# hpc4cmb/toast

Hardware: NVIDIA B200
Metric: detector-samples/s per destriper PCG iteration (higher is better)
Workload: dtype f64

## Files before the change

### include/toast_b200.h

```cpp
#ifndef TOAST_B200_H
#define TOAST_B200_H

#include <stddef.h>
#include <stdint.h>

#ifdef __cplusplus
extern "C" {
#endif

typedef struct {
    double start;
    double stop;
    int64_t first;
    int64_t last;
} tb_interval;

enum { TB_MEM_HOST = 0, TB_MEM_DEVICE = 1, TB_MEM_TABLE = 2 };

enum {
    TB_OK = 0,
    TB_ERR_CUDA = 1,
    TB_ERR_NO_DEVICE = 2,
    TB_ERR_ARG = 3,
    TB_ERR_NOT_PRESENT = 4,
// ... 186 lines not shown
    int64_t step_length;
    int64_t nside, n_pix_submap, n_submap;
    int nest, IAU;
    const int64_t *global2local;
    const double *boresight;
    const uint8_t *shared_flags;
    uint8_t shared_flag_mask;
    const uint8_t *solver_flags;
    uint8_t solver_flag_mask;
    const int64_t *pixels;
    const double *weights;
    const double *hwp;
} tb_obs_desc;

tb_obs *tb_obs_create(const tb_obs_desc *desc);
void tb_obs_destroy(tb_obs *obs);

int tb_lhs_pass1(const tb_obs *obs, const double *amplitudes, const uint8_t *amp_flags,
                 double *zmap, int regen, void *stream);
int tb_lhs_pass2(const tb_obs *obs, const double *amplitudes, const uint8_t *amp_flags,
                 const double *binned, double *amplitudes_out, int regen, void *stream);
int tb_obs_sorted_passes(const tb_obs *obs);
int tb_obs_set_pixel_chunks(tb_obs *obs, int64_t n_chunks, const int64_t *pixel_bounds);
int tb_lhs_pass1_chunk(const tb_obs *obs, const double *amplitudes, const uint8_t *amp_flags,
                       double *zmap, int64_t chunk, void *stream);
int tb_lhs_pass2_chunk(const tb_obs *obs, const double *binned, double *amplitudes_out,
                       int64_t chunk, void *stream);
int tb_lhs_pass2_cov(const tb_obs *obs, const double *zmap, const double *cov,
                     double *amplitudes_out, void *stream);
int tb_bx_block_pixels(void);
int tb_obs_blocked(const tb_obs *obs);
int tb_obs_blocked_stats(const tb_obs *obs, int64_t *n_records, int64_t *n_units,
                         int64_t *n_multi_units, int64_t *n_blocks);
int tb_bx_pass1(const tb_obs *obs, const double *amplitudes, const uint8_t *amp_flags,
                double *zmap, int accumulate, int64_t chunk, void *stream);
int tb_bx_pass2(const tb_obs *obs, const double *binned, double *amplitudes_out, int64_t chunk,
                void *stream);
int tb_bx_fused(const tb_obs *obs, const double *amplitudes, const uint8_t *amp_flags,
                const double *cov, double *zmap_scratch, double *amplitudes_out, void *stream);
int tb_rhs_project(const tb_obs *obs, const double *signal, const uint8_t *amp_flags,
                   const double *binned, double *amplitudes_out, int regen, void *stream);
int tb_bin_signal(const tb_obs *obs, const double *signal, double *zmap, int regen,
                  void *stream);

#define TB_PRECOND_TOEPLITZ 1
#define TB_PRECOND_BANDED 2
typedef struct {
    int64_t n_amp;
    int64_t n_seg;
    const int64_t *seg_start;
    const int64_t *seg_len;
    const int64_t *filt_start;
    const int64_t *filt_len;
    const double *filters;
    int64_t n_filter_values;
    int precond_mode;
    const int64_t *prec_start;
    const int64_t *prec_width;
    const double *precond;
    int64_t n_precond_values;
} tb_offset_prior_desc;
typedef struct tb_offset_prior tb_offset_prior;
tb_offset_prior *tb_offset_prior_create(const tb_offset_prior_desc *desc);
void tb_offset_prior_destroy(tb_offset_prior *prior);
int tb_offset_prior_add(const tb_offset_prior *prior, const double *amplitudes_in,
                        const uint8_t *amplitude_flags, double *amplitudes_out, int mem,
// ... 43 lines not shown
```

### toast_b200/csrc/tb_blocked.cu

```cuda
#include <algorithm>

#include "tb_obs.cuh"

using namespace tbd;

namespace tbr {
void sort_pairs_i32(const int32_t *keys_in, int32_t *keys_out, const int32_t *vals_in,
                    int32_t *vals_out, int64_t n, int end_bit, cudaStream_t st);
}

int g_use_bx = 1;

namespace {

#ifndef TB_BX_SHIFT
#define TB_BX_SHIFT 7
#endif
#ifndef TB_BX_CTAS
#define TB_BX_CTAS 4
#endif

constexpr int kBxShift = TB_BX_SHIFT;
constexpr int kBxPix = 1 << kBxShift;
constexpr int kBxUnitMax = 16384;
constexpr int kBxRowBits = 32 - (kBxShift + 12);
static_assert(kBxRowBits >= 1, "pixel | n0 | n1 must fit one int");

template <bool TWO_SLOT>
__global__ void __launch_bounds__(kThreads)
k_bx_keys(const int4 *__restrict__ xrec, int64_t n_rec, int32_t n_blocks, int32_t *__restrict__ keys,
          int32_t *__restrict__ vals, unsigned int *__restrict__ counters ) {
    for (int64_t i = (int64_t)blockIdx.x * kThreads + threadIdx.x; i < n_rec;
         i += (int64_t)gridDim.x * kThreads) {
        const int4 r = xrec[i];
        int32_t key = n_blocks, val = (int32_t)i, key2 = n_blocks, val2 = (int32_t)i | (2 << 30);
        if (r.x == -2 || r.y == -2) atomicAdd(counters + 2, 1u);
        if (r.x >= 0) {
            key = r.x >> kBxShift;
            if (r.y >= 0 && r.y != r.x) {
                val |= (1 << 30);
                key2 = r.y >> kBxShift;
                atomicAdd(counters, 1u);
            }
        } else if (r.y >= 0) {
// ... 61 lines not shown
        const double a0 = g0 ? __ldg(amps + o0 + i) * w0 : 0.0;
        if (paired) {
            const bool g1 = has1 && __ldg(aflags + o1 + i) == 0;
            const double a1 = g1 ? __ldg(amps + o1 + i) * w1 : 0.0;
            double2 *dst = reinterpret_cast<double2 *>(ascaled) + 2 * ((int64_t)row * nad + i);
            dst[0] = make_double2(a0, a1);
            dst[1] = make_double2(g0 ? w0 : 0.0, g1 ? w1 : 0.0);
        } else {
            reinterpret_cast<double2 *>(ascaled)[(int64_t)row * nad + i] =
                make_double2(a0, g0 ? w0 : 0.0);
        }
    }
}

struct BxArgs {
    const int4 *units;
    const int2 *brec;
    const double2 *bqu;
    const double *ascaled;
    double *out;
    const int64_t *amp_offsets;
    int32_t nad, n_det;
    double4 cst;
    const double4 *table;
    double inv_nad;
    int64_t n_pix;
    double *zmap;
    const double *cov;
    int accumulate;
};

constexpr int kBxWarps = kThreads / 32;

struct BxRec {
    int2 r;
    double2 qu;
};
template <bool KEEP_IN_L2>
__device__ __forceinline__ BxRec bx_load(const BxArgs &a, int i, int end, int lane) {
    BxRec x;
    x.r = make_int2(0, -1 - lane);
    x.qu = make_double2(0.0, 0.0);
    if (i < end) {
        x.r = KEEP_IN_L2 ? __ldg(a.brec + i) : __ldcs(a.brec + i);
        x.qu = KEEP_IN_L2 ? __ldg(a.bqu + i) : __ldcs(a.bqu + i);
    }
    return x;
}

struct BxAmp {
    double2 t;
    double2 w;
};
template <bool PAIRED, bool NEED_W>
__device__ __forceinline__ BxAmp bx_gather(const BxArgs &a, int32_t slot) {
    BxAmp g;
    g.t = g.w = make_double2(0.0, 0.0);
    if (slot >= 0) {
        if (PAIRED) {
            const double2 *p = reinterpret_cast<const double2 *>(a.ascaled) + 2 * (int64_t)slot;
            g.t = __ldg(p);
            if (NEED_W) g.w = __ldg(p + 1);
        } else {
            const double2 v = __ldg(reinterpret_cast<const double2 *>(a.ascaled) + slot);
            g.t.x = v.x;
            g.w.x = v.y;
        }
    }
    return g;
}

template <bool UNIFORM>
__device__ __forceinline__ double4 bx_consts(const BxArgs &a, int32_t slot) {
    if (UNIFORM) return a.cst;
    const int row = (int)fast_div((int64_t)(slot < 0 ? 0 : slot), a.inv_nad);
    const double2 *tp = reinterpret_cast<const double2 *>(a.table + row);
    const double2 ca = __ldg(tp), cb = __ldg(tp + 1);
    return make_double4(ca.x, ca.y, cb.x, cb.y);
}

template <bool UNIFORM, bool PAIRED>
__device__ __forceinline__ void bx_acc_step(const BxArgs &a, double *tile, const BxRec &x,
                                            const BxAmp &g, int lane) {
    const int p = x.r.x & (kBxPix - 1);
    const int n0 = (x.r.x >> kBxShift) & 63, n1 = (x.r.x >> (kBxShift + 6)) & 63;
    const double4 c = bx_consts<UNIFORM>(a, x.r.y);
    const double t0 = n0 ? g.t.x : 0.0;
    const double t1 = (PAIRED && n1) ? g.t.y : 0.0;
    const bool contrib = t0 != 0.0 || t1 != 0.0;
    const double v0 = t0 * (c.x * (double)n0) + t1 * (c.y * (double)n1);
    const double v1 = t0 * x.qu.x + t1 * (c.z * x.qu.x - c.w * x.qu.y);
    const double v2 = t0 * x.qu.y + t1 * (c.w * x.qu.x + c.z * x.qu.y);
    const unsigned same = __match_any_sync(0xffffffffu, contrib ? p : kBxPix + lane);
    const int rank = __popc(same & ((1u << lane) - 1u));
    const int rounds = __reduce_max_sync(0xffffffffu, rank);
    double *z = tile + 3 * p;
    if (rounds == 0) {
        if (contrib) {
            z[0] += v0;
            z[1] += v1;
            z[2] += v2;
        }
        __syncwarp();
    } else {
        for (int r = 0; r <= rounds; ++r) {
            if (contrib && rank == r) {
                z[0] += v0;
                z[1] += v1;
                z[2] += v2;
            }
            __syncwarp();
        }
    }
}

template <bool UNIFORM, bool PAIRED, bool KEEP_IN_L2>
__device__ __forceinline__ void bx_accumulate(const BxArgs &a, double *tile, int first, int end,
                                              int lane) {
    if (first >= end) return;
    BxRec A = bx_load<KEEP_IN_L2>(a, first + lane, end, lane);
    BxRec B = bx_load<KEEP_IN_L2>(a, first + 32 + lane, end, lane);
    BxRec C;
    BxAmp gA = bx_gather<PAIRED, false>(a, A.r.y), gB, gC;
    for (int base = first; base < end; base += 96) {
        C = bx_load<KEEP_IN_L2>(a, base + 64 + lane, end, lane);
        gB = bx_gather<PAIRED, false>(a, B.r.y);
        bx_acc_step<UNIFORM, PAIRED>(a, tile, A, gA, lane);
        if (base + 32 >= end) break;
        A = bx_load<KEEP_IN_L2>(a, base + 96 + lane, end, lane);
        gC = bx_gather<PAIRED, false>(a, C.r.y);
        bx_acc_step<UNIFORM, PAIRED>(a, tile, B, gB, lane);
        if (base + 64 >= end) break;
        B = bx_load<KEEP_IN_L2>(a, base + 128 + lane, end, lane);
        gA = bx_gather<PAIRED, false>(a, A.r.y);
        bx_acc_step<UNIFORM, PAIRED>(a, tile, C, gC, lane);
    }
}

template <bool UNIFORM, bool PAIRED>
__device__ __forceinline__ void bx_proj_step(const BxArgs &a, const double *tile, const BxRec &x,
                                             const BxAmp &g, int lane) {
    const int p = x.r.x & (kBxPix - 1);
    const int n0 = (x.r.x >> kBxShift) & 63, n1 = (x.r.x >> (kBxShift + 6)) & 63;
    const double4 c = bx_consts<UNIFORM>(a, x.r.y);
    const double m0 = tile[3 * p], m1 = tile[3 * p + 1], m2 = tile[3 * p + 2];
    double val0 = 0.0, val1 = 0.0;
    if (n0) {
        double sc = (c.x * (double)n0) * m0;
        sc += x.qu.x * m1;
        sc += x.qu.y * m2;
        val0 = (double)n0 * g.t.x - sc * g.w.x;
    }
    if (PAIRED && n1) {
        const double q1 = c.z * x.qu.x - c.w * x.qu.y, u1 = c.w * x.qu.x + c.z * x.qu.y;
        double sc = (c.y * (double)n1) * m0;
        sc += q1 * m1;
        sc += u1 * m2;
        val1 = (double)n1 * g.t.y - sc * g.w.y;
    }
    const Runs rr = find_runs32<8>(x.r.y, lane);
    val0 = seg_sum<8>(val0, rr);
    if (PAIRED) val1 = seg_sum<8>(val1, rr);
    if (rr.is_tail && x.r.y >= 0) {
        const int row = (int)((unsigned)x.r.x >> (kBxShift + 12));
        const int arel = x.r.y - row * a.nad;
        const int d0 = PAIRED ? 2 * row : row;
        if (val0 != 0.0) atomicAdd(a.out + __ldg(a.amp_offsets + d0) + arel, val0);
        if (PAIRED && val1 != 0.0) atomicAdd(a.out + __ldg(a.amp_offsets + d0 + 1) + arel, val1);
    }
}

template <bool UNIFORM, bool PAIRED>
__device__ __forceinline__ void bx_project(const BxArgs &a, const double *tile, int first, int end,
                                           int lane) {
    if (first >= end) return;
    BxRec A = bx_load<false>(a, first + lane, end, lane);
    BxRec B = bx_load<false>(a, first + 32 + lane, end, lane);
    BxRec C;
    BxAmp gA = bx_gather<PAIRED, true>(a, A.r.y), gB, gC;
    for (int base = first; base < end; base += 96) {
        C = bx_load<false>(a, base + 64 + lane, end, lane);
        gB = bx_gather<PAIRED, true>(a, B.r.y);
        bx_proj_step<UNIFORM, PAIRED>(a, tile, A, gA, lane);
        if (base + 32 >= end) break;
        A = bx_load<false>(a, base + 96 + lane, end, lane);
        gC = bx_gather<PAIRED, true>(a, C.r.y);
        bx_proj_step<UNIFORM, PAIRED>(a, tile, B, gB, lane);
        if (base + 64 >= end) break;
        B = bx_load<false>(a, base + 128 + lane, end, lane);
        gA = bx_gather<PAIRED, true>(a, A.r.y);
        bx_proj_step<UNIFORM, PAIRED>(a, tile, C, gC, lane);
    }
}

template <int MODE, bool UNIFORM, bool PAIRED>
__global__ void __launch_bounds__(kThreads, TB_BX_CTAS)
k_bx(const BxArgs a, int64_t n_units) {
    __shared__ __align__(16) double tiles[kBxWarps][3 * kBxPix];
    const int warp = threadIdx.x >> 5, lane = threadIdx.x & 31;
    double *tile = tiles[warp];
    double2 *tile2 = reinterpret_cast<double2 *>(tile);
    const int64_t g_end = 3 * a.n_pix;
    {
        const int64_t ticket = (int64_t)blockIdx.x * kBxWarps + warp;
        if (ticket >= n_units) return;
        const int4 u = __ldg(a.units + ticket);
        const int64_t g0 = (int64_t)u.x * (3 * kBxPix);
        if constexpr (MODE == 1) {
            if (u.z <= u.y) return;
            const double2 *src = reinterpret_cast<const double2 *>(a.zmap + g0);
#pragma unroll 4
            for (int k = lane; k < 3 * kBxPix / 2; k += 32) {
                const int64_t g = g0 + 2 * k;
                double2 v = make_double2(0.0, 0.0);
                if (g + 1 < g_end) v = __ldcs(src + k);
                else if (g < g_end) v.x = __ldcs(a.zmap + g);
                tile2[k] = v;
            }
            __syncwarp();
            bx_project<UNIFORM, PAIRED>(a, tile, u.y, u.z, lane);
        } else {
#pragma unroll 4
            for (int k = lane; k < 3 * kBxPix / 2; k += 32) tile2[k] = make_double2(0.0, 0.0);
            __syncwarp();
            bx_accumulate<UNIFORM, PAIRED, MODE == 2>(a, tile, u.y, u.z, lane);
            __syncwarp();
            if constexpr (MODE == 0) {
                if (u.w == 0 && !a.accumulate) {
                    double2 *dst = reinterpret_cast<double2 *>(a.zmap + g0);
#pragma unroll 4
                    for (int k = lane; k < 3 * kBxPix / 2; k += 32) {
                        const int64_t gg = g0 + 2 * k;
                        if (gg + 1 < g_end) __stcs(dst + k, tile2[k]);
                        else if (gg < g_end) a.zmap[gg] = tile2[k].x;
                    }
                } else {
                    for (int k = lane; k < 3 * kBxPix; k += 32) {
                        const double v = tile[k];
                        if (v != 0.0 && g0 + k < g_end) atomicAdd(a.zmap + g0 + k, v);
                    }
                }
            } else if (u.z > u.y) {
                for (int p = lane; p < kBxPix; p += 32) {
                    const int64_t gp = (int64_t)u.x * kBxPix + p;
                    const double z0 = tile[3 * p], z1 = tile[3 * p + 1], z2 = tile[3 * p + 2];
                    if (gp >= a.n_pix || (z0 == 0.0 && z1 == 0.0 && z2 == 0.0)) continue;
                    const double2 *cm = reinterpret_cast<const double2 *>(a.cov + 6 * gp);
                    const double2 ca = __ldcs(cm), cb = __ldcs(cm + 1), cc = __ldcs(cm + 2);
                    double m0 = 0.0, m1 = 0.0, m2 = 0.0;
                    m0 += ca.x * z0;
                    m0 += ca.y * z1;
                    m1 += ca.y * z0;
                    m0 += cb.x * z2;
                    m2 += cb.x * z0;
                    m1 += cb.y * z1;
                    m1 += cc.x * z2;
                    m2 += cc.x * z1;
                    m2 += cc.y * z2;
                    tile[3 * p] = m0;
                    tile[3 * p + 1] = m1;
                    tile[3 * p + 2] = m2;
                }
                __syncwarp();
                bx_project<UNIFORM, PAIRED>(a, tile, u.y, u.z, lane);
            }
        }
    }
}

__global__ void __launch_bounds__(kThreads)
k_bx_zero_blocks(const int32_t *__restrict__ blocks, int64_t n_pix, double *__restrict__ zmap) {
    const int64_t g0 = (int64_t)__ldg(blocks + blockIdx.x) * (3 * kBxPix);
    for (int k = threadIdx.x; k < 3 * kBxPix; k += kThreads)
        if (g0 + k < 3 * n_pix) zmap[g0 + k] = 0.0;
}

__global__ void __launch_bounds__(kThreads)
k_bx_cov_blocks(const int32_t *__restrict__ blocks, int64_t n_pix, const double *__restrict__ cov,
                double *__restrict__ zmap) {
    const int64_t p0 = (int64_t)__ldg(blocks + blockIdx.x) * kBxPix;
    for (int p = threadIdx.x; p < kBxPix; p += kThreads) {
        const int64_t gp = p0 + p;
        if (gp >= n_pix) continue;
        double *z = zmap + 3 * gp;
        const double z0 = z[0], z1 = z[1], z2 = z[2];
        const double *m = cov + 6 * gp;
        double t0 = 0.0, t1 = 0.0, t2 = 0.0;
        t0 += m[0] * z0;
        t0 += m[1] * z1;
        t1 += m[1] * z0;
        t0 += m[2] * z2;
        t2 += m[2] * z0;
        t1 += m[3] * z1;
        t1 += m[4] * z2;
        t2 += m[4] * z1;
        t2 += m[5] * z2;
        z[0] = t0;
        z[1] = t1;
        z[2] = t2;
    }
}

BxArgs make_args(const tb_obs *obs, const int4 *units) {
    BxArgs a;
    a.units = units;
    a.brec = obs->brec;
    a.bqu = obs->bqu;
    a.ascaled = obs->ascaled;
    a.out = nullptr;
    a.amp_offsets = obs->amp_offsets;
    a.nad = (int32_t)obs->n_amp_det;
    a.n_det = (int)obs->d.n_det;
    a.cst = make_double4(obs->s_const[0], obs->s_const[1], obs->s_const[2], obs->s_const[3]);
    a.table = obs->stable;
    a.inv_nad = 1.0 / (double)obs->n_amp_det;
    a.n_pix = obs->n_local_pix;
    a.zmap = nullptr;
    a.cov = nullptr;
    a.accumulate = 0;
    return a;
}

void row_grid(const tb_obs *obs, dim3 &grid) {
    int64_t gy = (obs->n_amp_det + kThreads * 4 - 1) / (kThreads * 4);
    if (gy < 1) gy = 1;
    if (gy > 65535) gy = 65535;
    grid = dim3((unsigned)obs->n_xrows, (unsigned)gy);
}

void launch_bx_prescale(const tb_obs *obs, const double *amps, const uint8_t *aflags, void *stream) {
    dim3 grid;
    row_grid(obs, grid);
    k_bx_prescale<<<grid, kThreads, 0, (cudaStream_t)stream>>>(
        obs->x_paired, (int)obs->d.n_det, obs->n_amp_det, obs->amp_offsets, obs->det_scale, amps,
        aflags, obs->ascaled);
    TB_CUDA(cudaGetLastError());
    tbr::count_launch();
}

template <int MODE>
void launch_bx(const tb_obs *obs, const BxArgs &a, int64_t n_units, void *stream) {
    if (n_units <= 0) return;
    const int64_t nb = (n_units + kBxWarps - 1) / kBxWarps;
    TB_REQUIRE(nb < 2147483647LL, "grid too large");
    const unsigned g = (unsigned)nb;
    cudaStream_t st = (cudaStream_t)stream;
    static bool configured = false;
    if (!configured) {
        auto prep = [&](const void *f) {
            TB_CUDA(cudaFuncSetAttribute(f, cudaFuncAttributePreferredSharedMemoryCarveout,
                                         (int)cudaSharedmemCarveoutMaxShared));
        };
        prep((const void *)k_bx<MODE, true, true>);
        prep((const void *)k_bx<MODE, true, false>);
        prep((const void *)k_bx<MODE, false, true>);
        prep((const void *)k_bx<MODE, false, false>);
        configured = true;
    }
    if (obs->s_uniform) {
        if (obs->x_paired) k_bx<MODE, true, true><<<g, kThreads, 0, st>>>(a, n_units);
        else k_bx<MODE, true, false><<<g, kThreads, 0, st>>>(a, n_units);
    } else {
        if (obs->x_paired) k_bx<MODE, false, true><<<g, kThreads, 0, st>>>(a, n_units);
        else k_bx<MODE, false, false><<<g, kThreads, 0, st>>>(a, n_units);
    }
    TB_CUDA(cudaGetLastError());
    tbr::count_launch();
}

inline bool bx_ok(const tb_obs *obs) { return g_use_bx && obs != nullptr && obs->brec != nullptr; }

void chunk_units(const tb_obs *obs, int64_t chunk, int64_t &first, int64_t &end) {
    first = 0;
    end = obs->n_bunits;
    if (chunk < 0) return;
    TB_REQUIRE(chunk + 1 < (int64_t)obs->bchunk_unit.size(),
               "bad chunk index (or pixel chunk bounds not aligned to the block size)");
    first = obs->bchunk_unit[chunk];
    end = obs->bchunk_unit[chunk + 1];
}

}

void tb_free_blocked(tb_obs *obs) {
    if (obs->brec) cudaFree(obs->brec);
    if (obs->bqu) cudaFree(obs->bqu);
    if (obs->bunits) cudaFree(obs->bunits);
    if (obs->bunits_single) cudaFree(obs->bunits_single);
    if (obs->bunits_multi) cudaFree(obs->bunits_multi);
    if (obs->bmulti_blocks) cudaFree(obs->bmulti_blocks);
    if (obs->ascaled) cudaFree(obs->ascaled);
    obs->ascaled = nullptr;
    obs->brec = nullptr;
    obs->bqu = nullptr;
    obs->bunits = obs->bunits_single = obs->bunits_multi = nullptr;
    obs->bmulti_blocks = nullptr;
    obs->n_brec = obs->n_bunits = obs->n_bunits_single = obs->n_bunits_multi = 0;
// ... 122 lines not shown
    for (int64_t c = 0; c <= n_chunks; ++c) {
        const int64_t b = pixel_bounds[c];
        if (!(b % kBxPix == 0 || b >= obs->n_local_pix)) {
            obs->bchunk_unit.clear();
            return;
        }
        const int64_t blk = (b + kBxPix - 1) >> kBxShift;
        auto it = std::lower_bound(obs->bunits_host.begin(), obs->bunits_host.end(), blk,
                                   [](const int4 &u, int64_t v) { return (int64_t)u.x < v; });
        cu[c] = (int64_t)(it - obs->bunits_host.begin());
    }
    cu[0] = 0;
    cu[n_chunks] = obs->n_bunits;
    obs->bchunk_unit = cu;
}

extern "C" {

int tb_bx_block_pixels(void) { return kBxPix; }

int tb_obs_blocked(const tb_obs *obs) { return bx_ok(obs) ? 1 : 0; }

int tb_obs_blocked_stats(const tb_obs *obs, int64_t *n_records, int64_t *n_units,
                         int64_t *n_multi_units, int64_t *n_blocks) {
    TB_API_BEGIN
    TB_REQUIRE(obs != nullptr, "NULL observation");
    if (n_records) *n_records = obs->n_brec;
    if (n_units) *n_units = obs->n_bunits;
    if (n_multi_units) *n_multi_units = obs->n_bunits_multi;
    if (n_blocks) *n_blocks = obs->brec ? (obs->n_local_pix + kBxPix - 1) >> kBxShift : 0;
    TB_API_END
}

int tb_bx_pass1(const tb_obs *obs, const double *amplitudes, const uint8_t *amp_flags,
                double *zmap, int accumulate, int64_t chunk, void *stream) {
    TB_API_BEGIN
    tbr::require_device();
    TB_REQUIRE(obs && amplitudes && amp_flags && zmap, "NULL argument");
    TB_REQUIRE(bx_ok(obs), "the observation has no block-ordered crossing list");
    TB_REQUIRE((reinterpret_cast<uintptr_t>(zmap) & 15u) == 0, "zmap must be 16-byte aligned");
    int64_t first, end;
    chunk_units(obs, chunk, first, end);
    if (chunk <= 0) launch_bx_prescale(obs, amplitudes, amp_flags, stream);
    if (!accumulate && obs->n_bmulti_blocks > 0 && chunk <= 0) {
        k_bx_zero_blocks<<<(unsigned)obs->n_bmulti_blocks, kThreads, 0, (cudaStream_t)stream>>>(
            obs->bmulti_blocks, obs->n_local_pix, zmap);
        TB_CUDA(cudaGetLastError());
        tbr::count_launch();
    }
    BxArgs a = make_args(obs, obs->bunits + first);
    a.zmap = zmap;
    a.accumulate = accumulate;
    launch_bx<0>(obs, a, end - first, stream);
    TB_API_END
}

int tb_bx_pass2(const tb_obs *obs, const double *binned, double *amplitudes_out, int64_t chunk,
                void *stream) {
    TB_API_BEGIN
    tbr::require_device();
    TB_REQUIRE(obs && binned && amplitudes_out, "NULL argument");
    TB_REQUIRE(bx_ok(obs), "the observation has no block-ordered crossing list");
    TB_REQUIRE((reinterpret_cast<uintptr_t>(binned) & 15u) == 0, "map must be 16-byte aligned");
    int64_t first, end;
    chunk_units(obs, chunk, first, end);
    BxArgs a = make_args(obs, obs->bunits + first);
// ... 45 lines not shown
```

### toast_b200/csrc/tb_obs.cuh

```cuda
#pragma once

#include <vector>

#include "tb_device.cuh"
#include "tb_runtime.cuh"

using tbd::Views;

struct tb_obs {
    void *blob = nullptr;
    Views V;
    const int64_t *amp_view_off = nullptr;
    const int64_t *amp_offsets = nullptr;
    const int64_t *g2l = nullptr;
    const double *fp = nullptr;
    const double *cal = nullptr;
    const double *eta = nullptr;
    const double *gamma = nullptr;
    const double *det_scale = nullptr;
    tb_obs_desc d;
    int64_t n_amp_det = 0;
    int64_t *tiles = nullptr;
    int64_t n_tiles = 0;
    int32_t *lpix = nullptr;
// ... 8 lines not shown
    int4 *srec = nullptr;
    double2 *squ = nullptr;
    double4 *stable = nullptr;
    double *dscaled = nullptr;
    int64_t n_srec = 0;
    int s_pass2_ok = 0;
    std::vector<int64_t> chunk_rec;
    double *ascaled = nullptr;
    int2 *brec = nullptr;
    double2 *bqu = nullptr;
    int4 *bunits = nullptr;
    int4 *bunits_single = nullptr, *bunits_multi = nullptr;
    int32_t *bmulti_blocks = nullptr;
    int64_t n_brec = 0, n_bunits = 0, n_bunits_single = 0, n_bunits_multi = 0, n_bmulti_blocks = 0;
    int64_t n_local_pix = 0;
    std::vector<int4> bunits_host;
    std::vector<int64_t> bchunk_unit;
    int s_uniform = 0;
    double s_const[4] = {0, 0, 0, 0};
};


constexpr unsigned long long kAmpFlagBits = 0x7FF8000000B200B2ULL;
__device__ __forceinline__ bool amp_is_flagged(double v) {
    return (unsigned long long)__double_as_longlong(v) == kAmpFlagBits;
}

void tb_launch_prescale(const tb_obs *obs, const double *amps, const uint8_t *aflags, void *stream);
void tb_build_row_table(tb_obs *obs);
void tb_build_blocked(tb_obs *obs, cudaStream_t st);
void tb_free_blocked(tb_obs *obs);
void tb_blocked_set_chunks(tb_obs *obs, int64_t n_chunks, const int64_t *pixel_bounds);
extern int g_use_bx;
```

### toast_b200/csrc/tb_solver.cu

```cuda
#include "tb_device.cuh"
#include "tb_runtime.cuh"

using namespace tbd;

#include "tb_obs.cuh"
#include "tb_tma.cuh"

namespace {

struct ObsDev {
    Views V;
    int64_t n_det, n_samp;
    const int64_t *amp_view_off, *amp_offsets, *g2l;
    const double *fp, *cal, *eta, *gamma, *det_scale;
    double inv_step, inv_nps;
    int64_t n_pix_submap;
    tbm::PixCtx ctx;
    double U_sign;
    const double *boresight;
    const uint8_t *shared_flags;
    uint8_t shared_mask;
    const uint8_t *solver_flags;
    uint8_t solver_mask;
    const int64_t *pixels;
// ... 1954 lines not shown
        }
        build_crossings(obs, (cudaStream_t)stream);
    }
    TB_API_END
}

int tb_obs_crossing_stats(const tb_obs *obs, int64_t *n_records, int64_t *n_rows, int *paired) {
    TB_API_BEGIN
    TB_REQUIRE(obs != nullptr, "NULL observation");
    if (n_records) *n_records = obs->xrec ? obs->n_xrec : 0;
    if (n_rows) *n_rows = obs->xrec ? obs->n_xrows : 0;
    if (paired) *paired = obs->xrec ? obs->x_paired : 0;
    TB_API_END
}

int tb_obs_has_compact_pointing(const tb_obs *obs) { return (obs && obs->lpix) ? 1 : 0; }
int tb_obs_has_pair_weights(const tb_obs *obs) { return (obs && obs->lpp) ? 1 : 0; }

extern int tb_peer_ctas_per_sm;
extern int tb_prior_chunk;

int tb_get_option(const char *name) {
    if (name == nullptr) return -1;
    std::string n(name);
    if (n == "tma") return g_use_tma;
    if (n == "compact") return g_use_compact;
    if (n == "pair") return g_use_pair;
    if (n == "pairw") return g_use_pairw;
    if (n == "crossings") return g_use_x;
    if (n == "sorted") return g_use_xs;
    if (n == "sorted2") return g_use_xs2;
    if (n == "peer_ctas") return tb_peer_ctas_per_sm;
    if (n == "blocked") return g_use_bx;
    if (n == "prior_chunk") return tb_prior_chunk;
    return -1;
}

int tb_set_option(const char *name, int value) {
    TB_API_BEGIN
    TB_REQUIRE(name != nullptr, "NULL option name");
    if (std::string(name) == "tma") {
        g_use_tma = value;
    } else if (std::string(name) == "compact") {
        g_use_compact = value;
    } else if (std::string(name) == "pair") {
        g_use_pair = value;
    } else if (std::string(name) == "pairw") {
        g_use_pairw = value;
    } else if (std::string(name) == "crossings") {
        g_use_x = value;
    } else if (std::string(name) == "sorted") {
        g_use_xs = value;
    } else if (std::string(name) == "sorted2") {
        g_use_xs2 = value;
    } else if (std::string(name) == "blocked") {
        g_use_bx = value;
    } else if (std::string(name) == "prior_chunk") {
        TB_REQUIRE(value >= 0, "prior_chunk must be >= 0");
        tb_prior_chunk = value;
    } else if (std::string(name) == "peer_ctas") {
        TB_REQUIRE(value >= 1 && value <= 16, "peer_ctas must be in [1, 16]");
        tb_peer_ctas_per_sm = value;
    } else {
        throw tbr::Error{TB_ERR_ARG, std::string("unknown option: ") + name};
    }
    TB_API_END
}

int tb_lhs_pass1(const tb_obs *obs, const double *amplitudes, const uint8_t *amp_flags,
                 double *zmap, int regen, void *stream) {
    TB_API_BEGIN
    tbr::require_device();
    TB_REQUIRE(obs && amplitudes && amp_flags && zmap, "NULL argument");
    launch_bin<false>(obs, amplitudes, amp_flags, nullptr, zmap, regen, stream);
    TB_API_END
}

int tb_lhs_pass2(const tb_obs *obs, const double *amplitudes, const uint8_t *amp_flags,
                 const double *binned, double *amplitudes_out, int regen, void *stream) {
    TB_API_BEGIN
    tbr::require_device();
    TB_REQUIRE(obs && amp_flags && binned && amplitudes_out, "NULL argument");
    launch_project<false>(obs, amplitudes, amp_flags, nullptr, binned, amplitudes_out, regen,
                          stream);
    TB_API_END
}

int tb_obs_sorted_passes(const tb_obs *obs) {
    if (obs == nullptr) return 0;
// ... 128 lines not shown
```

### toast_b200/lib.py

```python

import ctypes as ct
import os

import numpy as np

HERE = os.path.dirname(os.path.abspath(__file__))
LIB_PATH = os.environ.get("TB_LIB_PATH", os.path.join(HERE, "libtoastb200.so"))

TB_MEM_HOST, TB_MEM_DEVICE, TB_MEM_TABLE = 0, 1, 2
TB_ERR_NO_DEVICE = 2

interval_dtype = np.dtype(
    {
        "names": ["start", "stop", "first", "last"],
        "formats": ["d", "d", "q", "q"],
        "offsets": [0, 8, 16, 24],
    }
)

P = ct.c_void_p
I64 = ct.c_int64
I32 = ct.c_int32
U8 = ct.c_uint8
F64 = ct.c_double
# ... 65 lines not shown
    "tb_stokes_weights_I": (INT, [P, P, I64, P, I64, P, I64, I64, INT, P]),
    "tb_pointing_fused": (INT, [P, P, P, U8, P, P, I64, P, P, I64, P, P, I64, P, P, I64, P, I64,
                                I64, I64, INT, P, P, P, INT, I64, I64, INT, P]),
    "tb_noise_weight": (INT, [P, I64, P, P, I64, P, I64, I64, INT, P]),
    "tb_build_noise_weighted": (INT, [P, I64, P, I64, I64, I64, P, P, I64, P, P, I64, P, P, I64,
                                      P, P, I64, P, U8, P, I64, P, U8, I64, I64, INT, P]),
    "tb_scan_map": (INT, [P, I64, I64, P, INT, I64, I64, P, I64, P, P, I64, P, P, I64, P, P,
                          I64, F64, INT, INT, INT, I64, I64, INT, P]),
    "tb_template_offset_add_to_signal": (INT, [I64, I64, P, P, P, I64, I32, P, I64, P, I64, I64,
                                               INT, P]),
    "tb_template_offset_project_signal": (INT, [I32, P, I64, I32, P, I64, U8, I64, I64, P, P, P,
                                                I64, P, I64, I64, INT, P]),
    "tb_template_offset_apply_diag_precond": (INT, [P, P, P, P, I64, INT, P]),
    "tb_template_offset_add_to_signal_batch": (INT, [I64, P, P, P, P, I64, P, P, I64, P, I64,
                                                     I64, I64, INT, P]),
    "tb_template_offset_project_signal_batch": (INT, [P, P, I64, P, P, I64, U8, I64, P, P, P, P,
                                                      I64, P, I64, I64, I64, INT, P]),
    "tb_cov_apply_diag": (INT, [I64, I64, I64, P, P, INT, P]),
    "tb_cov_accum": (INT, [P, I64, I64, I64, I64, P, P, P, P, I64, P, P, I64, P, P, I64, P, U8,
                           P, I64, P, U8, I64, I64, INT, P]),
    "tb_cov_invert": (INT, [I64, I64, P, P, F64, INT, P]),
    "tb_obs_create": (P, [ct.POINTER(tb_obs_desc)]),
    "tb_obs_destroy": (None, [P]),
    "tb_lhs_pass1": (INT, [P, P, P, P, INT, P]),
    "tb_lhs_pass2": (INT, [P, P, P, P, P, INT, P]),
    "tb_obs_sorted_passes": (INT, [P]),
    "tb_obs_set_pixel_chunks": (INT, [P, I64, P]),
    "tb_lhs_pass1_chunk": (INT, [P, P, P, P, I64, P]),
    "tb_lhs_pass2_chunk": (INT, [P, P, P, I64, P]),
    "tb_lhs_pass2_cov": (INT, [P, P, P, P, P]),
    "tb_bx_block_pixels": (INT, []),
    "tb_obs_blocked": (INT, [P]),
    "tb_obs_blocked_stats": (INT, [P, P, P, P, P]),
    "tb_bx_pass1": (INT, [P, P, P, P, INT, I64, P]),
    "tb_bx_pass2": (INT, [P, P, P, I64, P]),
    "tb_bx_fused": (INT, [P, P, P, P, P, P, P]),
    "tb_rhs_project": (INT, [P, P, P, P, P, INT, P]),
    "tb_bin_signal": (INT, [P, P, P, INT, P]),
    "tb_offset_prior_create": (P, [ct.POINTER(tb_offset_prior_desc)]),
    "tb_offset_prior_destroy": (None, [P]),
    "tb_offset_prior_add": (INT, [P, P, P, P, INT, P]),
    "tb_offset_prior_precond": (INT, [P, P, P, P, INT, P]),
    "tb_peer_create": (P, [INT, INT, SZ]),
    "tb_peer_get_handles": (INT, [P, P]),
    "tb_peer_open": (INT, [P, P]),
    "tb_peer_map_ptr": (P, [P]),
    "tb_map_reduce_cov": (INT, [P, I64, P, P]),
    "tb_map_reduce_cov_range": (INT, [P, I64, I64, P, P]),
    "tb_peer_destroy": (None, [P]),
    "tb_peer_attach": (P, [INT, INT, SZ, P, P, ct.c_uint64]),
    "tb_peer_has_multicast": (INT, [P]),
    "tb_peer_set_multimem": (INT, [INT]),
    "tb_amp_dot": (INT, [P, P, P, I64, P, P]),
    "tb_pcg_update": (INT, [P, P, P, P, P, P, P, P, P, I64, P, P]),
    "tb_pcg_direction": (INT, [P, P, P, P, I64, P]),
    "tb_obs_pack_pointing": (INT, [P, P]),
    "tb_obs_has_compact_pointing": (INT, [P]),
    "tb_obs_has_pair_weights": (INT, [P]),
    "tb_obs_crossing_stats": (INT, [P, P, P, P]),
    "tb_set_option": (INT, [STR, INT]),
    "tb_get_option": (INT, [STR]),
    "tb_set_pixel_guard_scale": (None, [F64]),
    "tb_pixel_exact_count": (I64, [INT]),
}

_lib = None
# ... 72 lines not shown
```

Before: 303.5 billion.

## Split blocked shared-memory tile into I and QU arrays, add optional per-lane-parity copies

Result: faster. 308.0 billion (median of 6 runs) (+1.5%).

```diff
diff --git a/include/toast_b200.h b/include/toast_b200.h
--- a/include/toast_b200.h
+++ b/include/toast_b200.h
@@ -242,6 +242,9 @@
 int tb_obs_blocked(const tb_obs *obs);
 int tb_obs_blocked_stats(const tb_obs *obs, int64_t *n_records, int64_t *n_units,
                          int64_t *n_multi_units, int64_t *n_blocks);
+int tb_obs_blocked_step_stats(const tb_obs *obs, int copies, int64_t *n_steps,
+                              int64_t *sum_rounds, int64_t *n_red_sites);
+int tb_bx_fused_ctas_per_sm(const tb_obs *obs, int copies, int *ctas);
 int tb_bx_pass1(const tb_obs *obs, const double *amplitudes, const uint8_t *amp_flags,
                 double *zmap, int accumulate, int64_t chunk, void *stream);
 int tb_bx_pass2(const tb_obs *obs, const double *binned, double *amplitudes_out, int64_t chunk,
diff --git a/profiles/bx_tile_ab.py b/profiles/bx_tile_ab.py
--- /dev/null
+++ b/profiles/bx_tile_ab.py
@@ -0,0 +1,120 @@
+
+import argparse
+import ctypes as ct
+import json
+import os
+import subprocess
+import sys
+
+import numpy as np
+
+ROOT = os.path.dirname(os.path.dirname(os.path.abspath(__file__)))
+sys.path.insert(0, ROOT)
+
+import bench
+
+
+def card():
+    q = "name,power.limit,clocks.max.sm"
+    out = subprocess.run(["nvidia-smi", f"--query-gpu={q}", "--format=csv,noheader", "--id=0"],
+                         capture_output=True, text=True).stdout.strip()
+    return dict(zip(q.split(","), [x.strip() for x in out.split(",")]))
+
+
+def step_stats(lib, h, copies):
+    from toast_b200 import lib as L
+
+    n, r, red = ct.c_int64(0), ct.c_int64(0), ct.c_int64(0)
+    L.check(lib.tb_obs_blocked_step_stats(h, copies, ct.byref(n), ct.byref(r), ct.byref(red)))
+    c = ct.c_int(0)
+    L.check(lib.tb_bx_fused_ctas_per_sm(h, copies, ct.byref(c)))
+    return {"n_steps": n.value, "sum_rounds": r.value, "n_red_sites": red.value,
+            "rounds_per_step": r.value / max(n.value, 1),
+            "red_sites_per_step": red.value / max(n.value, 1), "fused_ctas_per_sm": c.value}
+
+
+def shard(workload, rounds, device, lib, steps, warmup):
+    import torch
+
+    from toast_b200 import lib as L
+
+    ds, dobs, signal, info = bench.build_gpu_problem(workload, False, 1.0, 0, 1, device)
+    h = dobs.handle().h
+    res = {"config": f"{workload}: {info['n_det']} det x {info['n_samp']} samples, nside "
+                     f"{info['nside']}", "setup_ms": info["setup_ms"],
+           "path": bench.describe_path(ds, dobs, lib, False, 1)[0]}
+    if not ds._blocked():
+        return res
+    st, sq0 = bench.pcg_prologue(ds, signal, lib)
+    for c in (1, 2):
+        L.check(lib.tb_set_option(b"bx_tile_copies", c))
+        res[f"copies{c}"] = {"stats": step_stats(lib, h, c), "kernel_ms": [], "step_ms": []}
+    lhs = {}
+    for c in (1, 2):
+        L.check(lib.tb_set_option(b"bx_tile_copies", c))
+        q = torch.zeros_like(st.d)
+        ds.lhs(st.d, q)
+        lhs[c] = q.cpu().numpy()
+    scale = float(np.max(np.abs(lhs[1])))
+    res["lhs_max_abs_diff_over_max_abs"] = float(np.max(np.abs(lhs[2] - lhs[1]))) / scale
+    for r in range(rounds):
+        for c in (1, 2):
+            L.check(lib.tb_set_option(b"bx_tile_copies", c))
+            ms, _, _ = bench.time_iterations(ds, st, sq0, steps, warmup, 1, lib)
+            k = bench.time_dominant_kernel(ds, dobs, st, lib, True, ds.fuse_lhs, reps=20)
+            res[f"copies{c}"]["step_ms"].append(ms)
+            res[f"copies{c}"]["kernel_ms"].append(k)
+    for c in (1, 2):
+        e = res[f"copies{c}"]
+        for key in ("step_ms", "kernel_ms"):
+            v = [x for x in e[key] if x is not None]
+            e[key + "_median"] = float(np.median(v)) if v else None
+            e[key + "_range"] = [float(min(v)), float(max(v))] if v else None
+    del ds, dobs, signal, st
+    torch.cuda.empty_cache()
+    return res
+
+
+def main():
+    ap = argparse.ArgumentParser()
+    ap.add_argument("--rounds", type=int, default=5, help="alternations on the C4 shard")
+    ap.add_argument("--other-rounds", type=int, default=2, help="alternations on C2, C3, C5")
+    ap.add_argument("--steps", type=int, default=50)
+    ap.add_argument("--warmup", type=int, default=5)
+    ap.add_argument("--out", default=os.path.join(ROOT, "profiles", "bx_tile_ab.json"))
+    args = ap.parse_args()
+
+    import torch
+
+    from toast_b200 import lib as L
+
+    lib = L.load()
+    device = torch.device("cuda", 0)
+    torch.cuda.set_device(device)
+    default = lib.tb_get_option(b"bx_tile_copies")
+    out = {"card": card(), "default_copies": default, "steps": args.steps,
+           "warmup": args.warmup, "shards": {}}
+    print(json.dumps(out["card"]), flush=True)
+    try:
+        for wl, rounds in (("c4", args.rounds), ("c2", args.other_rounds),
+                           ("c3", args.other_rounds), ("c5", args.other_rounds)):
+            r = shard(wl, rounds, device, lib, args.steps, args.warmup)
+            out["shards"][wl] = r
+            if "copies1" not in r:
+                print(json.dumps({"shard": wl, "path": r["path"]}), flush=True)
+                continue
+            summary = {c: {k: r[f"copies{c}"][k] for k in ("kernel_ms_median", "kernel_ms_range",
+                                                          "step_ms_median", "step_ms_range")}
+                       for c in (1, 2)}
+            stats = {c: r[f"copies{c}"]["stats"] for c in (1, 2)}
+            print(json.dumps({"shard": wl, "timing": summary, "stats": stats,
+                              "lhs_rel_diff": r["lhs_max_abs_diff_over_max_abs"]}), flush=True)
+    finally:
+        lib.tb_set_option(b"bx_tile_copies", default)
+    with open(args.out, "w") as f:
+        json.dump(out, f, indent=1)
+    print(f"wrote {args.out}")
+
+
+if __name__ == "__main__":
+    main()
diff --git a/toast_b200/csrc/tb_blocked.cu b/toast_b200/csrc/tb_blocked.cu
--- a/toast_b200/csrc/tb_blocked.cu
+++ b/toast_b200/csrc/tb_blocked.cu
@@ -10,6 +10,7 @@
 }
 
 int g_use_bx = 1;
+int g_bx_copies = 1;
 
 namespace {
 
@@ -137,6 +138,14 @@
 
 constexpr int kBxWarps = kThreads / 32;
 
+__device__ __forceinline__ int bx_swz_i(int c, int p) { return c * kBxPix + (p ^ (c << 3)); }
+__device__ __forceinline__ int bx_swz_qu(int c, int p) { return c * kBxPix + (p ^ (c << 2)); }
+
+__device__ __forceinline__ double &bx_tile_at(double *ti, double2 *tqu, int j) {
+    const int p = j / 3, k = j - 3 * p;
+    return k == 0 ? ti[p] : (k == 1 ? tqu[p].x : tqu[p].y);
+}
+
 struct BxRec {
     int2 r;
     double2 qu;
@@ -184,9 +193,9 @@
     return make_double4(ca.x, ca.y, cb.x, cb.y);
 }
 
-template <bool UNIFORM, bool PAIRED>
-__device__ __forceinline__ void bx_acc_step(const BxArgs &a, double *tile, const BxRec &x,
-                                            const BxAmp &g, int lane) {
+template <int COPIES, bool UNIFORM, bool PAIRED>
+__device__ __forceinline__ void bx_acc_step(const BxArgs &a, double *ti, double2 *tqu,
+                                            const BxRec &x, const BxAmp &g, int lane) {
     const int p = x.r.x & (kBxPix - 1);
     const int n0 = (x.r.x >> kBxShift) & 63, n1 = (x.r.x >> (kBxShift + 6)) & 63;
     const double4 c = bx_consts<UNIFORM>(a, x.r.y);
@@ -196,32 +205,62 @@
     const double v0 = t0 * (c.x * (double)n0) + t1 * (c.y * (double)n1);
     const double v1 = t0 * x.qu.x + t1 * (c.z * x.qu.x - c.w * x.qu.y);
     const double v2 = t0 * x.qu.y + t1 * (c.w * x.qu.x + c.z * x.qu.y);
-    const unsigned same = __match_any_sync(0xffffffffu, contrib ? p : kBxPix + lane);
+    const int copy = lane % COPIES;
+    const unsigned same =
+        __match_any_sync(0xffffffffu, contrib ? copy * kBxPix + p : COPIES * kBxPix + lane);
     const int rank = __popc(same & ((1u << lane) - 1u));
     const int rounds = __reduce_max_sync(0xffffffffu, rank);
-    double *z = tile + 3 * p;
+    double *zi = ti + bx_swz_i(copy, p);
+    double2 *zqu = tqu + bx_swz_qu(copy, p);
+    auto rmw = [&]() {
+        *zi += v0;
+        double2 z = *zqu;
+        z.x += v1;
+        z.y += v2;
+        *zqu = z;
+    };
+#ifdef TB_BX_AGG
+    (void)rank;
+    double s0 = v0, s1 = v1, s2 = v2;
+    const unsigned above = same & ~((2u << lane) - 1u);
+    int next = above ? __ffs(above) - 1 : -1;
+    for (int span = 1; span <= rounds; span <<= 1) {
+        const int src = next < 0 ? lane : next;
+        const double u0 = __shfl_sync(0xffffffffu, s0, src);
+        const double u1 = __shfl_sync(0xffffffffu, s1, src);
+        const double u2 = __shfl_sync(0xffffffffu, s2, src);
+        const int nn = __shfl_sync(0xffffffffu, next, src);
+        if (next >= 0) {
+            s0 += u0;
+            s1 += u1;
+            s2 += u2;
+            next = nn;
+        }
+    }
+    if (contrib && (same & ((1u << lane) - 1u)) == 0) {
+        *zi += s0;
+        double2 z = *zqu;
+        z.x += s1;
+        z.y += s2;
+        *zqu = z;
+    }
+    __syncwarp();
+#else
     if (rounds == 0) {
-        if (contrib) {
-            z[0] += v0;
-            z[1] += v1;
-            z[2] += v2;
-        }
+        if (contrib) rmw();
         __syncwarp();
     } else {
         for (int r = 0; r <= rounds; ++r) {
-            if (contrib && rank == r) {
-                z[0] += v0;
-                z[1] += v1;
-                z[2] += v2;
-            }
+            if (contrib && rank == r) rmw();
             __syncwarp();
         }
     }
-}
-
-template <bool UNIFORM, bool PAIRED, bool KEEP_IN_L2>
-__device__ __forceinline__ void bx_accumulate(const BxArgs &a, double *tile, int first, int end,
-                                              int lane) {
+#endif
+}
+
+template <int COPIES, bool UNIFORM, bool PAIRED, bool KEEP_IN_L2>
+__device__ __forceinline__ void bx_accumulate(const BxArgs &a, double *ti, double2 *tqu, int first,
+                                              int end, int lane) {
     if (first >= end) return;
     BxRec A = bx_load<KEEP_IN_L2>(a, first + lane, end, lane);
     BxRec B = bx_load<KEEP_IN_L2>(a, first + 32 + lane, end, lane);
@@ -230,25 +269,27 @@
     for (int base = first; base < end; base += 96) {
         C = bx_load<KEEP_IN_L2>(a, base + 64 + lane, end, lane);
         gB = bx_gather<PAIRED, false>(a, B.r.y);
-        bx_acc_step<UNIFORM, PAIRED>(a, tile, A, gA, lane);
+        bx_acc_step<COPIES, UNIFORM, PAIRED>(a, ti, tqu, A, gA, lane);
         if (base + 32 >= end) break;
         A = bx_load<KEEP_IN_L2>(a, base + 96 + lane, end, lane);
         gC = bx_gather<PAIRED, false>(a, C.r.y);
-        bx_acc_step<UNIFORM, PAIRED>(a, tile, B, gB, lane);
+        bx_acc_step<COPIES, UNIFORM, PAIRED>(a, ti, tqu, B, gB, lane);
         if (base + 64 >= end) break;
         B = bx_load<KEEP_IN_L2>(a, base + 128 + lane, end, lane);
         gA = bx_gather<PAIRED, false>(a, A.r.y);
-        bx_acc_step<UNIFORM, PAIRED>(a, tile, C, gC, lane);
+        bx_acc_step<COPIES, UNIFORM, PAIRED>(a, ti, tqu, C, gC, lane);
     }
 }
 
 template <bool UNIFORM, bool PAIRED>
-__device__ __forceinline__ void bx_proj_step(const BxArgs &a, const double *tile, const BxRec &x,
-                                             const BxAmp &g, int lane) {
+__device__ __forceinline__ void bx_proj_step(const BxArgs &a, const double *ti, const double2 *tqu,
+                                             const BxRec &x, const BxAmp &g, int lane) {
     const int p = x.r.x & (kBxPix - 1);
     const int n0 = (x.r.x >> kBxShift) & 63, n1 = (x.r.x >> (kBxShift + 6)) & 63;
     const double4 c = bx_consts<UNIFORM>(a, x.r.y);
-    const double m0 = tile[3 * p], m1 = tile[3 * p + 1], m2 = tile[3 * p + 2];
+    const double m0 = ti[p];
+    const double2 mqu = tqu[p];
+    const double m1 = mqu.x, m2 = mqu.y;
     double val0 = 0.0, val1 = 0.0;
     if (n0) {
         double sc = (c.x * (double)n0) * m0;
@@ -276,8 +317,8 @@
 }
 
 template <bool UNIFORM, bool PAIRED>
-__device__ __forceinline__ void bx_project(const BxArgs &a, const double *tile, int first, int end,
-                                           int lane) {
+__device__ __forceinline__ void bx_project(const BxArgs &a, const double *ti, const double2 *tqu,
+                                           int first, int end, int lane) {
     if (first >= end) return;
     BxRec A = bx_load<false>(a, first + lane, end, lane);
     BxRec B = bx_load<false>(a, first + 32 + lane, end, lane);
@@ -286,25 +327,27 @@
     for (int base = first; base < end; base += 96) {
         C = bx_load<false>(a, base + 64 + lane, end, lane);
         gB = bx_gather<PAIRED, true>(a, B.r.y);
-        bx_proj_step<UNIFORM, PAIRED>(a, tile, A, gA, lane);
+        bx_proj_step<UNIFORM, PAIRED>(a, ti, tqu, A, gA, lane);
         if (base + 32 >= end) break;
         A = bx_load<false>(a, base + 96 + lane, end, lane);
         gC = bx_gather<PAIRED, true>(a, C.r.y);
-        bx_proj_step<UNIFORM, PAIRED>(a, tile, B, gB, lane);
+        bx_proj_step<UNIFORM, PAIRED>(a, ti, tqu, B, gB, lane);
         if (base + 64 >= end) break;
         B = bx_load<false>(a, base + 128 + lane, end, lane);
         gA = bx_gather<PAIRED, true>(a, A.r.y);
-        bx_proj_step<UNIFORM, PAIRED>(a, tile, C, gC, lane);
-    }
-}
-
-template <int MODE, bool UNIFORM, bool PAIRED>
+        bx_proj_step<UNIFORM, PAIRED>(a, ti, tqu, C, gC, lane);
+    }
+}
+
+template <int MODE, int COPIES, bool UNIFORM, bool PAIRED>
 __global__ void __launch_bounds__(kThreads, TB_BX_CTAS)
 k_bx(const BxArgs a, int64_t n_units) {
-    __shared__ __align__(16) double tiles[kBxWarps][3 * kBxPix];
+    static_assert(COPIES == 1 || (COPIES == 2 && MODE != 1), "pass 2 reads one copy");
+    __shared__ __align__(16) double2 tiles_qu[kBxWarps][COPIES * kBxPix];
+    __shared__ __align__(16) double tiles_i[kBxWarps][COPIES * kBxPix];
     const int warp = threadIdx.x >> 5, lane = threadIdx.x & 31;
-    double *tile = tiles[warp];
-    double2 *tile2 = reinterpret_cast<double2 *>(tile);
+    double *ti = tiles_i[warp];
+    double2 *tqu = tiles_qu[warp];
     const int64_t g_end = 3 * a.n_pix;
     {
         const int64_t ticket = (int64_t)blockIdx.x * kBxWarps + warp;
@@ -320,35 +363,55 @@
                 double2 v = make_double2(0.0, 0.0);
                 if (g + 1 < g_end) v = __ldcs(src + k);
                 else if (g < g_end) v.x = __ldcs(a.zmap + g);
-                tile2[k] = v;
+                bx_tile_at(ti, tqu, 2 * k) = v.x;
+                bx_tile_at(ti, tqu, 2 * k + 1) = v.y;
             }
             __syncwarp();
-            bx_project<UNIFORM, PAIRED>(a, tile, u.y, u.z, lane);
+            bx_project<UNIFORM, PAIRED>(a, ti, tqu, u.y, u.z, lane);
         } else {
+            double2 *ti2 = reinterpret_cast<double2 *>(ti);
 #pragma unroll 4
-            for (int k = lane; k < 3 * kBxPix / 2; k += 32) tile2[k] = make_double2(0.0, 0.0);
+            for (int k = lane; k < COPIES * kBxPix; k += 32) {
+                tqu[k] = make_double2(0.0, 0.0);
+                if (k < COPIES * kBxPix / 2) ti2[k] = make_double2(0.0, 0.0);
+            }
             __syncwarp();
-            bx_accumulate<UNIFORM, PAIRED, MODE == 2>(a, tile, u.y, u.z, lane);
+            bx_accumulate<COPIES, UNIFORM, PAIRED, MODE == 2>(a, ti, tqu, u.y, u.z, lane);
             __syncwarp();
+            if constexpr (COPIES == 2) {
+                for (int p = lane; p < kBxPix; p += 32) {
+                    ti[p] += ti[bx_swz_i(1, p)];
+                    double2 z = tqu[p];
+                    const double2 z1 = tqu[bx_swz_qu(1, p)];
+                    z.x += z1.x;
+                    z.y += z1.y;
+                    tqu[p] = z;
+                }
+                __syncwarp();
+            }
             if constexpr (MODE == 0) {
                 if (u.w == 0 && !a.accumulate) {
                     double2 *dst = reinterpret_cast<double2 *>(a.zmap + g0);
 #pragma unroll 4
                     for (int k = lane; k < 3 * kBxPix / 2; k += 32) {
                         const int64_t gg = g0 + 2 * k;
-                        if (gg + 1 < g_end) __stcs(dst + k, tile2[k]);
-                        else if (gg < g_end) a.zmap[gg] = tile2[k].x;
+                        const double2 v = make_double2(bx_tile_at(ti, tqu, 2 * k),
+                                                       bx_tile_at(ti, tqu, 2 * k + 1));
+                        if (gg + 1 < g_end) __stcs(dst + k, v);
+                        else if (gg < g_end) a.zmap[gg] = v.x;
                     }
                 } else {
                     for (int k = lane; k < 3 * kBxPix; k += 32) {
-                        const double v = tile[k];
+                        const double v = bx_tile_at(ti, tqu, k);
                         if (v != 0.0 && g0 + k < g_end) atomicAdd(a.zmap + g0 + k, v);
                     }
                 }
             } else if (u.z > u.y) {
                 for (int p = lane; p < kBxPix; p += 32) {
                     const int64_t gp = (int64_t)u.x * kBxPix + p;
-                    const double z0 = tile[3 * p], z1 = tile[3 * p + 1], z2 = tile[3 * p + 2];
+                    const double z0 = ti[p];
+                    const double2 zqu = tqu[p];
+                    const double z1 = zqu.x, z2 = zqu.y;
                     if (gp >= a.n_pix || (z0 == 0.0 && z1 == 0.0 && z2 == 0.0)) continue;
                     const double2 *cm = reinterpret_cast<const double2 *>(a.cov + 6 * gp);
                     const double2 ca = __ldcs(cm), cb = __ldcs(cm + 1), cc = __ldcs(cm + 2);
@@ -362,12 +425,11 @@
                     m1 += cc.x * z2;
                     m2 += cc.x * z1;
                     m2 += cc.y * z2;
-                    tile[3 * p] = m0;
-                    tile[3 * p + 1] = m1;
-                    tile[3 * p + 2] = m2;
+                    ti[p] = m0;
+                    tqu[p] = make_double2(m1, m2);
                 }
                 __syncwarp();
-                bx_project<UNIFORM, PAIRED>(a, tile, u.y, u.z, lane);
+                bx_project<UNIFORM, PAIRED>(a, ti, tqu, u.y, u.z, lane);
             }
         }
     }
@@ -406,6 +468,35 @@
     }
 }
 
+__global__ void __launch_bounds__(kThreads)
+k_bx_step_stats(const int4 *__restrict__ units, int64_t n_units, const int2 *__restrict__ brec,
+                int copies, unsigned long long *__restrict__ out ) {
+    const int lane = threadIdx.x & 31;
+    const int64_t ticket = (int64_t)blockIdx.x * kBxWarps + (threadIdx.x >> 5);
+    if (ticket >= n_units) return;
+    const int4 u = units[ticket];
+    unsigned long long steps = 0, rounds = 0, reds = 0;
+    for (int base = u.y; base < u.z; base += 32) {
+        const int i = base + lane;
+        const int2 r = i < u.z ? brec[i] : make_int2(0, -1 - lane);
+        const bool contrib = ((r.x >> kBxShift) & 4095) != 0;
+        const int c = lane % copies;
+        const unsigned same = __match_any_sync(
+            0xffffffffu, contrib ? c * kBxPix + (r.x & (kBxPix - 1)) : copies * kBxPix + lane);
+        const int rank = __popc(same & ((1u << lane) - 1u));
+        const Runs rr = find_runs32<8>(r.y, lane);
+        const unsigned tails = __ballot_sync(0xffffffffu, rr.is_tail && r.y >= 0);
+        steps += 1;
+        rounds += 1 + __reduce_max_sync(0xffffffffu, rank);
+        reds += __popc(tails);
+    }
+    if (lane == 0 && steps > 0) {
+        atomicAdd(out, steps);
+        atomicAdd(out + 1, rounds);
+        atomicAdd(out + 2, reds);
+    }
+}
+
 BxArgs make_args(const tb_obs *obs, const int4 *units) {
     BxArgs a;
     a.units = units;
@@ -443,6 +534,30 @@
     tbr::count_launch();
 }
 
+template <int MODE, int COPIES>
+void launch_bx_copies(const tb_obs *obs, const BxArgs &a, int64_t n_units, unsigned g,
+                      cudaStream_t st) {
+    static bool configured = false;
+    if (!configured) {
+        auto prep = [&](const void *f) {
+            TB_CUDA(cudaFuncSetAttribute(f, cudaFuncAttributePreferredSharedMemoryCarveout,
+                                         (int)cudaSharedmemCarveoutMaxShared));
+        };
+        prep((const void *)k_bx<MODE, COPIES, true, true>);
+        prep((const void *)k_bx<MODE, COPIES, true, false>);
+        prep((const void *)k_bx<MODE, COPIES, false, true>);
+        prep((const void *)k_bx<MODE, COPIES, false, false>);
+        configured = true;
+    }
+    if (obs->s_uniform) {
+        if (obs->x_paired) k_bx<MODE, COPIES, true, true><<<g, kThreads, 0, st>>>(a, n_units);
+        else k_bx<MODE, COPIES, true, false><<<g, kThreads, 0, st>>>(a, n_units);
+    } else {
+        if (obs->x_paired) k_bx<MODE, COPIES, false, true><<<g, kThreads, 0, st>>>(a, n_units);
+        else k_bx<MODE, COPIES, false, false><<<g, kThreads, 0, st>>>(a, n_units);
+    }
+}
+
 template <int MODE>
 void launch_bx(const tb_obs *obs, const BxArgs &a, int64_t n_units, void *stream) {
     if (n_units <= 0) return;
@@ -450,24 +565,11 @@
     TB_REQUIRE(nb < 2147483647LL, "grid too large");
     const unsigned g = (unsigned)nb;
     cudaStream_t st = (cudaStream_t)stream;
-    static bool configured = false;
-    if (!configured) {
-        auto prep = [&](const void *f) {
-            TB_CUDA(cudaFuncSetAttribute(f, cudaFuncAttributePreferredSharedMemoryCarveout,
-                                         (int)cudaSharedmemCarveoutMaxShared));
-        };
-        prep((const void *)k_bx<MODE, true, true>);
-        prep((const void *)k_bx<MODE, true, false>);
-        prep((const void *)k_bx<MODE, false, true>);
-        prep((const void *)k_bx<MODE, false, false>);
-        configured = true;
-    }
-    if (obs->s_uniform) {
-        if (obs->x_paired) k_bx<MODE, true, true><<<g, kThreads, 0, st>>>(a, n_units);
-        else k_bx<MODE, true, false><<<g, kThreads, 0, st>>>(a, n_units);
+    if constexpr (MODE != 1) {
+        if (g_bx_copies == 2) launch_bx_copies<MODE, 2>(obs, a, n_units, g, st);
+        else launch_bx_copies<MODE, 1>(obs, a, n_units, g, st);
     } else {
-        if (obs->x_paired) k_bx<MODE, false, true><<<g, kThreads, 0, st>>>(a, n_units);
-        else k_bx<MODE, false, false><<<g, kThreads, 0, st>>>(a, n_units);
+        launch_bx_copies<MODE, 1>(obs, a, n_units, g, st);
     }
     TB_CUDA(cudaGetLastError());
     tbr::count_launch();
@@ -656,6 +758,53 @@
     TB_API_END
 }
 
+int tb_obs_blocked_step_stats(const tb_obs *obs, int copies, int64_t *n_steps,
+                              int64_t *sum_rounds, int64_t *n_red_sites) {
+    TB_API_BEGIN
+    tbr::require_device();
+    TB_REQUIRE(obs != nullptr, "NULL observation");
+    TB_REQUIRE(copies == 1 || copies == 2, "copies must be 1 or 2");
+    TB_REQUIRE(obs->brec != nullptr, "the observation has no block-ordered crossing list");
+    unsigned long long h[3] = {0, 0, 0}, *d = nullptr;
+    TB_CUDA(cudaMalloc(&d, sizeof(h)));
+    cudaError_t e = cudaMemset(d, 0, sizeof(h));
+    if (e == cudaSuccess && obs->n_bunits > 0) {
+        k_bx_step_stats<<<(unsigned)((obs->n_bunits + kBxWarps - 1) / kBxWarps), kThreads>>>(
+            obs->bunits, obs->n_bunits, obs->brec, copies, d);
+        e = cudaGetLastError();
+        tbr::count_launch();
+    }
+    if (e == cudaSuccess) e = cudaMemcpy(h, d, sizeof(h), cudaMemcpyDeviceToHost);
+    cudaFree(d);
+    TB_CUDA(e);
+    if (n_steps) *n_steps = (int64_t)h[0];
+    if (sum_rounds) *sum_rounds = (int64_t)h[1];
+    if (n_red_sites) *n_red_sites = (int64_t)h[2];
+    TB_API_END
+}
+
+int tb_bx_fused_ctas_per_sm(const tb_obs *obs, int copies, int *ctas) {
+    TB_API_BEGIN
+    tbr::require_device();
+    TB_REQUIRE(obs != nullptr && ctas != nullptr, "NULL argument");
+    TB_REQUIRE(copies == 1 || copies == 2, "copies must be 1 or 2");
+    {
+        const void *f = copies == 2
+            ? (obs->s_uniform ? (obs->x_paired ? (const void *)k_bx<2, 2, true, true>
+                                               : (const void *)k_bx<2, 2, true, false>)
+                              : (obs->x_paired ? (const void *)k_bx<2, 2, false, true>
+                                               : (const void *)k_bx<2, 2, false, false>))
+            : (obs->s_uniform ? (obs->x_paired ? (const void *)k_bx<2, 1, true, true>
+                                               : (const void *)k_bx<2, 1, true, false>)
+                              : (obs->x_paired ? (const void *)k_bx<2, 1, false, true>
+                                               : (const void *)k_bx<2, 1, false, false>));
+        TB_CUDA(cudaFuncSetAttribute(f, cudaFuncAttributePreferredSharedMemoryCarveout,
+                                     (int)cudaSharedmemCarveoutMaxShared));
+        TB_CUDA(cudaOccupancyMaxActiveBlocksPerMultiprocessor(ctas, f, kThreads, 0));
+    }
+    TB_API_END
+}
+
 int tb_bx_pass1(const tb_obs *obs, const double *amplitudes, const uint8_t *amp_flags,
                 double *zmap, int accumulate, int64_t chunk, void *stream) {
     TB_API_BEGIN
diff --git a/toast_b200/csrc/tb_obs.cuh b/toast_b200/csrc/tb_obs.cuh
--- a/toast_b200/csrc/tb_obs.cuh
+++ b/toast_b200/csrc/tb_obs.cuh
@@ -64,3 +64,4 @@
 void tb_free_blocked(tb_obs *obs);
 void tb_blocked_set_chunks(tb_obs *obs, int64_t n_chunks, const int64_t *pixel_bounds);
 extern int g_use_bx;
+extern int g_bx_copies;
diff --git a/toast_b200/csrc/tb_solver.cu b/toast_b200/csrc/tb_solver.cu
--- a/toast_b200/csrc/tb_solver.cu
+++ b/toast_b200/csrc/tb_solver.cu
@@ -2010,6 +2010,7 @@
     if (n == "sorted2") return g_use_xs2;
     if (n == "peer_ctas") return tb_peer_ctas_per_sm;
     if (n == "blocked") return g_use_bx;
+    if (n == "bx_tile_copies") return g_bx_copies;
     if (n == "prior_chunk") return tb_prior_chunk;
     return -1;
 }
@@ -2033,6 +2034,9 @@
         g_use_xs2 = value;
     } else if (std::string(name) == "blocked") {
         g_use_bx = value;
+    } else if (std::string(name) == "bx_tile_copies") {
+        TB_REQUIRE(value == 1 || value == 2, "bx_tile_copies must be 1 or 2");
+        g_bx_copies = value;
     } else if (std::string(name) == "prior_chunk") {
         TB_REQUIRE(value >= 0, "prior_chunk must be >= 0");
         tb_prior_chunk = value;
diff --git a/toast_b200/lib.py b/toast_b200/lib.py
--- a/toast_b200/lib.py
+++ b/toast_b200/lib.py
@@ -121,6 +121,8 @@
     "tb_bx_block_pixels": (INT, []),
     "tb_obs_blocked": (INT, [P]),
     "tb_obs_blocked_stats": (INT, [P, P, P, P, P]),
+    "tb_obs_blocked_step_stats": (INT, [P, INT, P, P, P]),
+    "tb_bx_fused_ctas_per_sm": (INT, [P, INT, P]),
     "tb_bx_pass1": (INT, [P, P, P, P, INT, I64, P]),
     "tb_bx_pass2": (INT, [P, P, P, I64, P]),
     "tb_bx_fused": (INT, [P, P, P, P, P, P, P]),
```
